# exoplanet-dev/celerite2

Measured on AMD Instinct MI355X. Metric: float64 GP log-lik+grad/sec at N=4096 J=8, batched, higher is better.
Workload: dtype f64; 1 GPU; configs[2]: batch of 65536 independent GPs (65536 per GPU), N=4096, J=8 (sum of 4 SHO terms), forward + reverse-mode grad, inputs resident in HBM; global_batch=65536, batch_per_gpu=65536, N=4096, J=8, parallelism=batch-sharded x1, all-gather of log-liks, failed_factorizations=0, clock_prewarm_steps=0

## Files before the change

### celerite2_amd/csrc/c2_loglik_t.hip

```cpp
#include <cstdint>
#include <cstdlib>
#include <type_traits>

#include "c2_loglik_helpers.hpp"
#include "../../include/celerite2_amd.h"

#ifndef C2T_J
#define C2T_J 8
#endif
#ifndef C2T_JS
#define C2T_JS C2T_J
#endif
#define C2T_CAT2(a, b) a##b
#define C2T_CAT(a, b) C2T_CAT2(a, b)
#define C2T_NAME(stem) C2T_CAT(stem, C2T_JS)
#define c2t C2T_CAT(c2t_j, C2T_JS)

namespace c2t {
using namespace c2;

constexpr int J = C2T_J;
static_assert(J == 8 || J == 4 || J == 2, "128-byte tiles of whole rows");
constexpr int NS = J * (J + 1) / 2;
constexpr int PPR = J / 2;
// ... 49 lines not shown
  __device__ __forceinline__ int rl(int i) const { const int s = (kWave / LPS) * i + lane / LPS; return (FULL || s < last) ? s : last; }
};
using RowIO = RowIOT<false>;

typedef double d2v __attribute__((ext_vector_type(2)));
__device__ __forceinline__ double2 ld2_in(const double2 *p) {
  const d2v v = __builtin_nontemporal_load(reinterpret_cast<const d2v *>(p));
  return make_double2(v.x, v.y);
}
__device__ __forceinline__ double ld1_in(const double *p) { return __builtin_nontemporal_load(p); }
template <class IO>
__device__ __forceinline__ void row_fetch(const double *__restrict__ base, int64_t N, int64_t n0, const IO &io,
                                          double (&st)[2 * NI]) {
  int64_t r = n0 + io.rpiece / PPR;
  r = r < 0 ? 0 : (r > N - 1 ? N - 1 : r);
  const int pc = piece_in(io.rpiece) ? io.rpiece % PPR : 0;
  const int64_t off = r * JS + 2 * pc;
#pragma unroll
  for (int i = 0; i < NI; ++i) {
    const double2 v = ld2_in(reinterpret_cast<const double2 *>(base + (int64_t)io.rl(i) * N * JS + off));
    st[2 * i] = piece_in(io.rpiece) ? v.x : 0.0; st[2 * i + 1] = piece_in(io.rpiece) ? v.y : 0.0;
  }
}
__device__ __forceinline__ void row_stage(double *tile, int lane, const double (&st)[2 * NI]) {
#pragma unroll
  for (int i = 0; i < NI; ++i)
    *reinterpret_cast<double2 *>(tile + ((kWave / LPS) * i + lane / LPS) * RSTR + 2 * (lane % LPS)) =
        make_double2(st[2 * i], st[2 * i + 1]);
}
__device__ __forceinline__ void row_read(const double *tile, int lane, int r, double (&x)[J]) {
#pragma unroll
  for (int q = 0; q < J / 2; ++q) {
    const double2 v = *reinterpret_cast<const double2 *>(tile + lane * RSTR + r * J + 2 * q);
    x[2 * q] = v.x; x[2 * q + 1] = v.y;
  }
}
__device__ __forceinline__ void row_write(double *tile, int lane, int r, const double (&x)[J]) {
#pragma unroll
  for (int q = 0; q < J / 2; ++q)
    *reinterpret_cast<double2 *>(tile + lane * RSTR + r * J + 2 * q) = make_double2(x[2 * q], x[2 * q + 1]);
}
__device__ __forceinline__ void row_flush(double *__restrict__ base, int64_t N, int64_t n0, int64_t lo, int64_t hi,
                                          const double *tile, int lane, int last) {
  const int piece = lane % LPS;
  const int64_t r = n0 + piece / PPR;
  if (last == kWave - 1 && n0 >= lo && n0 + RT - 1 <= hi) {
#pragma unroll
    for (int i = 0; i < NI; ++i) {
      const int s = (kWave / LPS) * i + lane / LPS;
      if (piece_in(piece))
        *reinterpret_cast<double2 *>(base + (int64_t)s * N * JS + r * JS + 2 * (piece % PPR)) =
            *reinterpret_cast<const double2 *>(tile + s * RSTR + 2 * piece);
    }
    return;
  }
#pragma unroll
  for (int i = 0; i < NI; ++i) {
    const int s = (kWave / LPS) * i + lane / LPS;
    const double2 v = *reinterpret_cast<const double2 *>(tile + s * RSTR + 2 * piece);
    if (s <= last && r >= lo && r <= hi && piece_in(piece))
      *reinterpret_cast<double2 *>(base + (int64_t)s * N * JS + r * JS + 2 * (piece % PPR)) = v;
  }
}

__device__ __forceinline__ void row_flush_full(double *__restrict__ base, int64_t N, int64_t n0, const double *tile,
                                               int lane) {
  const int piece = lane % LPS;
  const int64_t off = (n0 + piece / PPR) * JS + 2 * (piece % PPR);
#pragma unroll
  for (int i = 0; i < NI; ++i) {
    const int s = (kWave / LPS) * i + lane / LPS;
    if (piece_in(piece))
      *reinterpret_cast<double2 *>(base + (int64_t)s * N * JS + off) =
          *reinterpret_cast<const double2 *>(tile + s * RSTR + 2 * piece);
  }
}

__device__ __forceinline__ void sc_fetch(const double *__restrict__ base, int64_t N, int64_t n0, const RowIO &io,
                                         double (&st)[8]) {
  int64_t r = n0 + io.piece;
  r = r < 0 ? 0 : (r > N - 1 ? N - 1 : r);
#pragma unroll
  for (int i = 0; i < 8; ++i) st[i] = base[(int64_t)io.sl(i) * N + r];
}
__device__ __forceinline__ void sc_stage(double *tile, int lane, const double (&st)[8]) {
#pragma unroll
  for (int i = 0; i < 8; ++i) tile[(8 * i + lane / 8) * SSTR + (lane & 7)] = st[i];
}
__device__ __forceinline__ void sc_fetch16(const double *__restrict__ base, int64_t sN, int64_t N, int64_t n16, int lane,
                                           int last, double (&st)[16]) {
  int64_t r = n16 + (lane & 15);
  r = r < 0 ? 0 : (r > N - 1 ? N - 1 : r);
#pragma unroll
  for (int i = 0; i < 16; ++i) {
    const int s = 4 * i + lane / 16;
    st[i] = ld1_in(&base[(int64_t)(s < last ? s : last) * sN + r]);
  }
}
__device__ __forceinline__ void sc_stage16(double *tile, int lane, int half, const double (&st)[16]) {
  if (((lane & 15) >> 3) == half) {
#pragma unroll
    for (int i = 0; i < 16; ++i) tile[(4 * i + lane / 16) * SSTR + (lane & 7)] = st[i];
  }
}
__device__ __forceinline__ void sc_flush(double *__restrict__ base, int64_t N, int64_t n0, int64_t lo, int64_t hi,
                                         const double *tile, int lane, int last) {
  const int64_t r = n0 + (lane & 7);
  if (last == kWave - 1 && n0 >= lo && n0 + ST - 1 <= hi) {
    double v[8];
#pragma unroll
    for (int i = 0; i < 8; ++i) v[i] = tile[(8 * i + lane / 8) * SSTR + (lane & 7)];
    __builtin_amdgcn_sched_barrier(0);
#pragma unroll
    for (int i = 0; i < 8; ++i) base[(int64_t)(8 * i + lane / 8) * N + r] = v[i];
    return;
  }
#pragma unroll
  for (int i = 0; i < 8; ++i) {
    const int s = 8 * i + lane / 8;
    const double v = tile[s * SSTR + (lane & 7)];
    if (s <= last && r >= lo && r <= hi) base[(int64_t)s * N + r] = v;
  }
}

__device__ __forceinline__ void apark(double x, int &lo, int &hi) {
  asm volatile("v_accvgpr_write_b32 %0, %1" : "=a"(lo) : "v"(__double2loint(x)));
  asm volatile("v_accvgpr_write_b32 %0, %1" : "=a"(hi) : "v"(__double2hiint(x)));
}
template <int IMM>
__device__ __forceinline__ void aload(int &dst, const double *sbase, unsigned voff) {
  asm volatile("global_load_dword %0, %1, %2 offset:%3 nt" : "=a"(dst) : "v"(voff), "s"(sbase), "n"(IMM));
}
__device__ __forceinline__ void await_aloads() { asm volatile("s_waitcnt vmcnt(0)" ::: "memory"); }
__device__ __forceinline__ double afetch(int lo, int hi) {
  int l, h;
  asm volatile("v_accvgpr_read_b32 %0, %1" : "=v"(l) : "a"(lo));
  asm volatile("v_accvgpr_read_b32 %0, %1" : "=v"(h) : "a"(hi));
  return __hiloint2double(h, l);
}

#ifndef C2T_MLDS
#define C2T_MLDS 0
#endif
__device__ __forceinline__ double2 ld2_stream(const double2 *p) {
  const d2v v = __builtin_nontemporal_load(reinterpret_cast<const d2v *>(p));
  return make_double2(v.x, v.y);
}
__device__ __forceinline__ double ld1_stream(const double *p) { return __builtin_nontemporal_load(p); }
__device__ __forceinline__ void st2_stream(double2 *p, double2 v) {
  d2v w; w.x = v.x; w.y = v.y;
  __builtin_nontemporal_store(w, reinterpret_cast<d2v *>(p));
}
__device__ __forceinline__ void st1_stream(double *p, double v) { __builtin_nontemporal_store(v, p); }

template <bool PAIRED>
__device__ __forceinline__ void decay(const double (&c)[J], double dt, double (&p)[J]) {
  if constexpr (PAIRED) {
#pragma unroll
    for (int k = 0; k < J / 2; ++k) p[2 * k] = p[2 * k + 1] = exp_decay(c[2 * k] * dt);
  } else {
#pragma unroll
    for (int j = 0; j < J; ++j) p[j] = exp_decay(c[j] * dt);
  }
}

#ifdef C2T_PROF
__device__ unsigned long long c2t_prof[8];
#define C2T_TICK(k)                                                    \
  do {                                                                 \
    __builtin_amdgcn_sched_barrier(0);                                 \
    const unsigned long long now_ = __builtin_readcyclecounter();      \
    prof_[k] += now_ - tick_;                                          \
    tick_ = now_;                                                      \
    __builtin_amdgcn_sched_barrier(0);                                 \
  } while (0)
#else
#define C2T_TICK(k) do {} while (0)
#endif

struct TermsArgs {
  const double *ar, *cr, *ac, *bc, *cc, *dc;
  int batched;
};
template <int JC>
struct TermCoef {
  static constexpr int JR = J - 2 * (JC > 0 ? JC : 0);
  double ar[JR > 0 ? JR : 1], ac[JC > 0 ? JC : 1], bc[JC > 0 ? JC : 1], dc[JC > 0 ? JC : 1], A0;
  __device__ __forceinline__ void load(const TermsArgs &T, int64_t b, double (&cj)[J]) {
    const int64_t br = T.batched ? b * JR : 0, bk = T.batched ? b * JC : 0;
    double sum = 0.0;
#pragma unroll
    for (int r = 0; r < JR; ++r) { ar[r] = T.ar[br + r]; cj[r] = T.cr[br + r]; sum += ar[r]; }
#pragma unroll
    for (int k = 0; k < JC; ++k) {
      ac[k] = T.ac[bk + k]; bc[k] = T.bc[bk + k]; dc[k] = T.dc[bk + k];
      cj[JR + 2 * k] = cj[JR + 2 * k + 1] = T.cc[bk + k];
      sum += ac[k];
    }
    A0 = sum;
  }
  template <bool FAST>
  static __device__ __forceinline__ void sc(double ph, double &sn, double &cs) {
    if constexpr (FAST) sincos_cw_fast(ph, sn, cs);
    else sincos(ph, &sn, &cs);
  }
  __device__ __forceinline__ bool phases_fast(double x_first, double x_last) const {
    const double xm = fmax(fabs(x_first), fabs(x_last));
    bool ok = true;
#pragma unroll
    for (int k = 0; k < JC; ++k) ok = ok && (fabs(dc[k]) * xm < kSincosFastMax);
    return ok;
  }
  template <bool FAST>
  __device__ __forceinline__ void rows(double xn, double (&u)[J], double (&v)[J]) const {
#pragma unroll
    for (int r = 0; r < JR; ++r) { u[r] = ar[r]; v[r] = 1.0; }
#pragma unroll
    for (int k = 0; k < JC; ++k) {
      double sn, cs;
      sc<FAST>(dc[k] * xn, sn, cs);
      v[JR + 2 * k] = cs; v[JR + 2 * k + 1] = sn;
      u[JR + 2 * k] = fma(ac[k], cs, bc[k] * sn);
      u[JR + 2 * k + 1] = fma(ac[k], sn, -(bc[k] * cs));
    }
  }
  template <bool FAST>
  __device__ __forceinline__ void rows_sc(double xn, double (&u)[J], double (&sn)[JC > 0 ? JC : 1],
                                          double (&cs)[JC > 0 ? JC : 1]) const {
#pragma unroll
    for (int r = 0; r < JR; ++r) u[r] = ar[r];
#pragma unroll
    for (int k = 0; k < JC; ++k) {
      sc<FAST>(dc[k] * xn, sn[k], cs[k]);
      u[JR + 2 * k] = fma(ac[k], cs[k], bc[k] * sn[k]);
      u[JR + 2 * k + 1] = fma(ac[k], sn[k], -(bc[k] * cs[k]));
    }
  }
  __device__ __forceinline__ void decay(const double (&cj)[J], double dt, double (&p)[J]) const {
#pragma unroll
    for (int r = 0; r < JR; ++r) p[r] = exp_decay(cj[r] * dt);
#pragma unroll
    for (int k = 0; k < JC; ++k) p[JR + 2 * k] = p[JR + 2 * k + 1] = exp_decay(cj[JR + 2 * k] * dt);
  }
};

template <bool REC, bool PAIRED, int JC = -1, bool FAST = true>
__device__ __forceinline__ void fwd_body(int64_t B, int64_t N, const double *__restrict__ t, int64_t t_bs,
                                         const double *__restrict__ c, int64_t c_bs, const double *__restrict__ a,
                                         const double *__restrict__ U, const double *__restrict__ V,
                                         const double *__restrict__ y, double *__restrict__ ll,
                                         int32_t *__restrict__ flag, double *__restrict__ rec, Rec R,
                                         unsigned long long *__restrict__ guard, double *lds,
                                         const TermsArgs T = TermsArgs{}) {
  constexpr bool TERMS = JC >= 0;
  const int lane = threadIdx.x;
  const int64_t b0 = (int64_t)blockIdx.x * kWave;
  const int last = (int)((B - 1 - b0) < (kWave - 1) ? (B - 1 - b0) : (kWave - 1));
  const int sl = lane < last ? lane : last;
  const int64_t b = b0 + sl;
  const RowIO io(lane, last);
  double *tU = lds, *tV = tU + kWave * RSTR, *tT = tV + kWave * RSTR, *tA = tT + kWave * SSTR, *tY = tA + kWave * SSTR;
  const double *Ub = U + b0 * N * JS, *Vb = V + b0 * N * JS, *ab = a + b0 * N, *yb = y + b0 * N;
  const double *tb = t + (t_bs ? b0 * N : 0);
  const int64_t tN = t_bs ? N : 0;

  double cj[J];
  TermCoef<JC> tc;
  if constexpr (TERMS) tc.load(T, b, cj);
  else {
#pragma unroll
    for (int j = 0; j < J; ++j) cj[j] = j < JS ? c[b * c_bs + j] : 0.0;
  }
  double cmax = 0.0;
#pragma unroll
  for (int j = 0; j < J; ++j) cmax = fmax(cmax, cj[j]);

  constexpr size_t rsW = (size_t)(J / 2) * kWave, rs1 = kWave;
  double2 *recW = REC ? reinterpret_cast<double2 *>(rec + R.w + (size_t)blockIdx.x * N * J * kWave) : nullptr;
  double2 *recDZ = REC ? reinterpret_cast<double2 *>(rec + R.dz + (size_t)blockIdx.x * N * 2 * kWave) : nullptr;
  double *recCK = REC ? rec + R.ck + (size_t)blockIdx.x * R.nck * (NS + J) * kWave : nullptr;
  int32_t *recCKR = REC ? reinterpret_cast<int32_t *>(rec + R.ckr + (size_t)blockIdx.x * (((size_t)N + 1) / 2)) : nullptr;
  double *recT = REC ? rec + R.t + (size_t)blockIdx.x * N * kWave : nullptr;

  double S[NS];
#pragma unroll
  for (int k = 0; k < NS; ++k) S[k] = 0.0;
  double F[J], w[J];
  double tprev = t[b * t_bs];
  double d = a[b * N], z = y[b * N];
  if constexpr (TERMS) d += tc.A0;
  double rd = 1.0 / d;
  if constexpr (TERMS) {
    double u0[J], v0[J];
    tc.template rows<FAST>(tprev, u0, v0);
#pragma unroll
    for (int j = 0; j < J; ++j) { F[j] = 0.0; w[j] = v0[j] * rd; }
  } else {
#pragma unroll
    for (int j = 0; j < J; ++j) { F[j] = 0.0; w[j] = j < JS ? V[b * N * JS + j] * rd : 0.0; }
  }
  double prod = d, quad = z * z * rd;
  int eacc = 0;
  int32_t fl = 0;
  int slot = 0, nextra = 0;
  int64_t lastck = 0;
  auto write_ckpt = [&](int64_t row) __attribute__((always_inline)) {
// ... 92 lines not shown
            for (int j2 = 0; j2 < J; ++j2) w[j2] = (v[j2] - tau[j2]) * rd;
            fl = ((fl == 0) & (d <= 0.0)) ? (int32_t)n : fl;
            prod *= d;
            quad = fma(z * z, rd, quad);
            if (r & 1) { int e; prod = frexp(prod, &e); eacc += e; }
            if (REC) {
#pragma unroll
              for (int q = 0; q < J / 2; ++q) st2_stream(&recW[(size_t)n * rsW + q * kWave + lane], make_double2(w[2 * q], w[2 * q + 1]));
              const bool seg_end = (n % C == 0) || (n == N - 1);
              st2_stream(&recDZ[(size_t)n * rs1 + lane], make_double2(seg_end ? -fabs(d) : fabs(d), z));
              st1_stream(&recT[(size_t)n * rs1 + lane], tn);
              if (seg_end) write_ckpt(n);
            }
          }
        }
      }
    }
  }
  if (lane <= last) {
    int e;
    prod = frexp(prod, &e);
    const double logdet = log(prod) + (double)(eacc + e) * kLn2;
    flag[b] = fl;
    ll[b] = fl ? -INFINITY : -0.5 * (logdet + (double)N * kLog2Pi) - 0.5 * quad;
    if (REC && lane == 0) recCKR[0] = nextra;
  }
  if (REC) {
    double g = (gmax == gmax) ? gmax : INFINITY;
#pragma unroll
    for (int sft = 1; sft < kWave; sft <<= 1) g = fmax(g, __shfl_xor(g, sft, kWave));
    if (lane == 0) {
      const unsigned long long bits = (unsigned long long)__double_as_longlong(g);
      guard[kGateHeadWords + blockIdx.x] = bits;
      atomicMax(guard, bits);
      if (g > kGuard) atomicAdd(guard + 1, 1ull);
    }
  }
}

constexpr int kFwdLds = (2 * kWave * RSTR + 3 * kWave * SSTR) * 8;

template <bool REC>
__global__ __launch_bounds__(kWave, 1) void k_loglik_t_fwd(int64_t B, int64_t N, const double *__restrict__ t,
                                                           int64_t t_bs, const double *__restrict__ c, int64_t c_bs,
                                                           const double *__restrict__ a, const double *__restrict__ U,
                                                           const double *__restrict__ V, const double *__restrict__ y,
                                                           double *__restrict__ ll, int32_t *__restrict__ flag,
                                                           double *__restrict__ rec, Rec R,
                                                           unsigned long long *__restrict__ guard) {
  __shared__ __attribute__((aligned(16))) double lds[kFwdLds / 8];
  const int lane = threadIdx.x;
  const int64_t b0 = (int64_t)blockIdx.x * kWave;
  const int64_t bb = (b0 + lane) < B ? (b0 + lane) : (B - 1);
  bool paired = true;
#pragma unroll
  for (int k = 0; k < JS / 2; ++k) paired = paired && (c[bb * c_bs + 2 * k] == c[bb * c_bs + 2 * k + 1]);
  if (__all(paired))
    fwd_body<REC, true>(B, N, t, t_bs, c, c_bs, a, U, V, y, ll, flag, rec, R, guard, lds);
  else
    fwd_body<REC, false>(B, N, t, t_bs, c, c_bs, a, U, V, y, ll, flag, rec, R, guard, lds);
}

template <int JC>
__device__ __forceinline__ bool terms_phases_fast(int64_t B, int64_t N, const double *__restrict__ x, int64_t x_bs,
                                                  const TermsArgs &T) {
  const int64_t b0 = (int64_t)blockIdx.x * kWave;
  const int64_t b = (b0 + threadIdx.x) < B ? (b0 + threadIdx.x) : (B - 1);
  TermCoef<JC> tc;
  double cj[J];
  tc.load(T, b, cj);
  return __all(tc.phases_fast(x[b * x_bs], x[b * x_bs + N - 1]));
}

template <int JC, bool REC>
__global__ __launch_bounds__(kWave, 1) void k_loglik_tt_fwd(int64_t B, int64_t N, const double *__restrict__ t,
                                                            int64_t t_bs, TermsArgs T, const double *__restrict__ diag,
                                                            const double *__restrict__ y, double *__restrict__ ll,
                                                            int32_t *__restrict__ flag, double *__restrict__ rec, Rec R,
                                                            unsigned long long *__restrict__ guard) {
  __shared__ __attribute__((aligned(16))) double lds[kFwdLds / 8];
  if (terms_phases_fast<JC>(B, N, t, t_bs, T))
    fwd_body<REC, true, JC, true>(B, N, t, t_bs, nullptr, 0, diag, nullptr, nullptr, y, ll, flag, rec, R, guard, lds, T);
  else
    fwd_body<REC, true, JC, false>(B, N, t, t_bs, nullptr, 0, diag, nullptr, nullptr, y, ll, flag, rec, R, guard, lds, T);
}

constexpr int RS1 = J + 2;
constexpr int CS4 = 6;
constexpr int kRevLds = (2 * kWave * RSTR + 3 * kWave * SSTR + kWave * CS4 + kWave * RS1) * 8;
static_assert(kRevLds <= 40960 && (kWave * RSTR + kWave * RS1 + 3 * kWave * SSTR + 2 * kWave * RS1) * 8 <= kRevLds, "four wavefronts per CU");

__device__ __forceinline__ void row1_read(const double *tile, int lane, double (&x)[J]) {
#pragma unroll
  for (int q = 0; q < J / 2; ++q) {
    const double2 v = *reinterpret_cast<const double2 *>(tile + lane * RS1 + 2 * q);
    x[2 * q] = v.x; x[2 * q + 1] = v.y;
  }
}
__device__ __forceinline__ void row1_write(double *tile, int lane, const double (&x)[J]) {
#pragma unroll
  for (int q = 0; q < J / 2; ++q)
    *reinterpret_cast<double2 *>(tile + lane * RS1 + 2 * q) = make_double2(x[2 * q], x[2 * q + 1]);
}
__device__ __forceinline__ void row1_flush(double *__restrict__ base, int64_t N, int64_t n, const double *tile, int lane,
                                           int last) {
#pragma unroll
  for (int i = 0; i < PPR; ++i) {
    int sr = (kWave / PPR) * i + lane / PPR; sr = sr < last ? sr : last;
    if (piece_in(lane % PPR))
      *reinterpret_cast<double2 *>(base + ((int64_t)sr * N + n) * JS + 2 * (lane % PPR)) =
          *reinterpret_cast<const double2 *>(tile + sr * RS1 + 2 * (lane % PPR));
  }
}

struct TermsGrads {
  double *bar, *bcr, *bac, *bbc, *bcc, *bdc;
};
constexpr int AS1 = 14;

template <int K, class Step>
__device__ __forceinline__ void for_phases(Step &step, int64_t ntop, int64_t nf) {
  if constexpr (K >= 0) {
    const int64_t m = ntop - (RT - 1 - K);
    if (m <= nf && m >= 1) step(m, std::integral_constant<int, K>{});
    for_phases<K - 1>(step, ntop, nf);
  }
}

template <bool PAIRED, int JC = -1, bool FAST = true, bool FULL = false, bool XCK = false>
__device__ __forceinline__ void rev_body(int64_t B, int64_t N, const double *__restrict__ t, int64_t t_bs,
                                         const double *__restrict__ c, int64_t c_bs, const double *__restrict__ U,
                                         const int32_t *__restrict__ flag, const double *__restrict__ rec, Rec R,
                                         double *__restrict__ bt, double *__restrict__ bc, double *__restrict__ ba,
                                         double *__restrict__ bU, double *__restrict__ bV, double *__restrict__ by,
                                         double *lds, const TermsArgs T = TermsArgs{}, const TermsGrads G = TermsGrads{}) {
  constexpr bool TERMS = JC >= 0;
  constexpr int JR = TermCoef<JC>::JR, JCN = JC > 0 ? JC : 1;
  constexpr int NACC = TERMS ? JR + 3 * JC + 1 : 1;
  static_assert(NACC <= AS1, "accumulator tile");
  const int lane = threadIdx.x;
  const int64_t b0 = (int64_t)blockIdx.x * kWave;
  const int last = (int)((B - 1 - b0) < (kWave - 1) ? (B - 1 - b0) : (kWave - 1));
  const int sl = lane < last ? lane : last;
  const int64_t b = b0 + sl;
  const RowIOT<FULL> io(lane, last);
  constexpr bool BVPAIR = PAIRED && !TERMS;
  constexpr int CSTR = BVPAIR ? CS4 : RS1;
  double *tU = lds, *tBV = tU + kWave * RSTR, *tBA = tBV + kWave * (BVPAIR ? RSTR : RS1), *tBY = tBA + kWave * SSTR,
         *tBT = tBY + kWave * SSTR, *tC = tBT + kWave * SSTR, *tBC = tC + kWave * CSTR;
  static_assert((kWave * RSTR + kWave * (BVPAIR ? RSTR : RS1) + 3 * kWave * SSTR + kWave * CSTR + kWave * RS1) * 8 <= kRevLds, "LDS");
  double *tACC = lds;
  const double *Ub = U + b0 * N * JS;
  double *bUb = bU + b0 * N * JS, *bVb = bV + b0 * N * JS, *bab = ba + b0 * N, *byb = by + b0 * N, *btb = bt + b0 * N;
  constexpr size_t rsW = (size_t)(J / 2) * kWave, rs1 = kWave;
  const double2 *recW = reinterpret_cast<const double2 *>(rec + R.w + (size_t)blockIdx.x * N * J * kWave);
  const double2 *recDZ = reinterpret_cast<const double2 *>(rec + R.dz + (size_t)blockIdx.x * N * 2 * kWave);
  const double *recCK = rec + R.ck + (size_t)blockIdx.x * R.nck * (NS + J) * kWave;
  const int32_t *recCKR = reinterpret_cast<const int32_t *>(rec + R.ckr + (size_t)blockIdx.x * (((size_t)N + 1) / 2));
  const double *recT = rec + R.t + (size_t)blockIdx.x * N * kWave;
  const bool failed = flag[b] != 0;
  const double nan = __builtin_nan("");

  TermCoef<JC> tc;
  {
    double cj[J], zero[J];
    if constexpr (TERMS) tc.load(T, b, cj);
    else {
#pragma unroll
      for (int j = 0; j < J; ++j) cj[j] = j < JS ? c[b * c_bs + j] : 0.0;
    }
#pragma unroll
    for (int j = 0; j < J; ++j) zero[j] = 0.0;
    if constexpr (BVPAIR) {
#pragma unroll
      for (int k = 0; k < PPR; k += 2)
        *reinterpret_cast<double2 *>(tC + lane * CS4 + k) = make_double2(cj[2 * k], cj[2 * k + 2 < J ? 2 * k + 2 : 2 * k]);
    } else {
      row1_write(tC, lane, cj);
    }
    row1_write(tBC, lane, zero);
    if constexpr (TERMS) {
#pragma unroll
      for (int q = 0; q < AS1 / 2; ++q) *reinterpret_cast<double2 *>(tACC + lane * AS1 + 2 * q) = make_double2(0.0, 0.0);
    }
  }
  auto read_rates = [&](double (&cj)[J]) __attribute__((always_inline)) {
    if constexpr (BVPAIR) {
#pragma unroll
      for (int k = 0; k < PPR; k += 2) {
        const double2 c2k = *reinterpret_cast<const double2 *>(tC + lane * CS4 + k);
        cj[2 * k] = cj[2 * k + 1] = c2k.x;
        if (2 * k + 2 < J) cj[2 * k + 2] = cj[2 * k + 3] = c2k.y;
      }
    } else {
      row1_read(tC, lane, cj);
    }
  };
  auto accumulate = [&](const double (&u)[J], const double (&bu)[J], const double (&sn)[JCN], const double (&cs)[JCN],
                        const double (&gv)[JCN], double ba_n, double xn) -> double {
    double acc[AS1];
#pragma unroll
    for (int q = 0; q < AS1 / 2; ++q) {
      const double2 v = *reinterpret_cast<const double2 *>(tACC + lane * AS1 + 2 * q);
      acc[2 * q] = v.x; acc[2 * q + 1] = v.y;
    }
    double gsum = 0.0;
#pragma unroll
    for (int r = 0; r < JR; ++r) acc[r] += bu[r];
#pragma unroll
    for (int k = 0; k < JC; ++k) {
      const double b0_ = bu[JR + 2 * k], b1_ = bu[JR + 2 * k + 1];
      acc[JR + 3 * k] = fma(b0_, cs[k], fma(b1_, sn[k], acc[JR + 3 * k]));
      acc[JR + 3 * k + 1] = fma(b0_, sn[k], fma(-b1_, cs[k], acc[JR + 3 * k + 1]));
      const double g = fma(-b0_, u[JR + 2 * k + 1], fma(b1_, u[JR + 2 * k], gv[k]));
      acc[JR + 3 * k + 2] = fma(g, xn, acc[JR + 3 * k + 2]);
      gsum = fma(g, tc.dc[k], gsum);
    }
    acc[NACC - 1] += ba_n;
#pragma unroll
    for (int q = 0; q < AS1 / 2; ++q)
      *reinterpret_cast<double2 *>(tACC + lane * AS1 + 2 * q) = make_double2(acc[2 * q], acc[2 * q + 1]);
    return gsum;
  };

  double F[J], bF[J], bVn[J];
  int Slo[NS], Shi[NS], Mlo[NS], Mhi[NS];
#pragma unroll
  for (int k = 0; k < NS; ++k) { apark(0.0, Slo[k], Shi[k]); apark(0.0, Mlo[k], Mhi[k]); }
  constexpr int NML = (TERMS && C2T_MLDS && NS >= 18) ? 18 : 0;
  auto mslot = [&](int q) -> double2 * {
    return reinterpret_cast<double2 *>(lds + (q < 7 ? kWave * AS1 + q * 2 * kWave : kRevLds / 8 - (9 - q) * 2 * kWave)) + lane;
  };
  static_assert(NML == 0 || kWave * AS1 + 7 * 2 * kWave <= kWave * RSTR + kWave * RS1, "free LDS behind the accumulator tile");
  if constexpr (NML > 0) {
#pragma unroll
    for (int q = 0; q < NML / 2; ++q) *mslot(q) = make_double2(0.0, 0.0);
  }
  double2 mpair = make_double2(0.0, 0.0);
#pragma unroll
  for (int j = 0; j < J; ++j) { F[j] = 0.0; bF[j] = 0.0; bVn[j] = failed ? nan : 0.0; }
  double carry = 0.0;

  const double2 dzl = recDZ[(size_t)(N - 1) * rs1 + lane];
  const double rdl = 1.0 / fabs(dzl.x);
  double ban = 0.5 * rdl * (dzl.y * dzl.y * rdl - 1.0), bzn = -dzl.y * rdl;
  if (failed) { ban = nan; bzn = nan; }
  double tcur = recT[(size_t)(N - 1) * rs1 + lane];

  auto load_ckpt = [&](int64_t row) {
    const int64_t slot = XCK ? (int64_t)__builtin_amdgcn_readfirstlane(recCKR[row])
                             : ((row % C == 0) ? row / C - 1 : R.nreg - 1);
    const double *ck = recCK + (size_t)slot * (NS + J) * kWave;
    const unsigned voff = (unsigned)lane * 8u;
#pragma unroll
    for (int k = 0; k < NS; ++k) {
      const double *base = ck + (k / 8) * 8 * kWave;
      if ((k & 7) == 0) { aload<0>(Slo[k], base, voff); aload<4>(Shi[k], base, voff); }
      if ((k & 7) == 1) { aload<512>(Slo[k], base, voff); aload<516>(Shi[k], base, voff); }
      if ((k & 7) == 2) { aload<1024>(Slo[k], base, voff); aload<1028>(Shi[k], base, voff); }
      if ((k & 7) == 3) { aload<1536>(Slo[k], base, voff); aload<1540>(Shi[k], base, voff); }
      if ((k & 7) == 4) { aload<2048>(Slo[k], base, voff); aload<2052>(Shi[k], base, voff); }
      if ((k & 7) == 5) { aload<2560>(Slo[k], base, voff); aload<2564>(Shi[k], base, voff); }
      if ((k & 7) == 6) { aload<3072>(Slo[k], base, voff); aload<3076>(Shi[k], base, voff); }
      if ((k & 7) == 7) { aload<3584>(Slo[k], base, voff); aload<3588>(Shi[k], base, voff); }
    }
#pragma unroll
    for (int j = 0; j < J; ++j) F[j] = ld1_stream(&ck[(NS + j) * kWave + lane]);
    await_aloads();
  };
  auto t_fetch = [&](int64_t row) { return ld1_stream(&recT[(size_t)(row < 0 ? 0 : row) * rs1 + lane]); };
  auto w_fetch = [&](int64_t row, double (&wv)[J]) {
    row = row < 0 ? 0 : row;
#pragma unroll
    for (int q = 0; q < J / 2; ++q) {
      const double2 v = ld2_stream(&recW[(size_t)row * rsW + q * kWave + lane]);
      wv[2 * q] = v.x; wv[2 * q + 1] = v.y;
    }
  };
  auto dz_fetch = [&](int64_t row) { return ld2_stream(&recDZ[(size_t)(row < 0 ? 0 : row) * rs1 + lane]); };

  if (N >= 2) {
    const int64_t nf = N - 1;
    const int ph0 = (int)(nf % RT);
    const bool bv_seed_waits = BVPAIR && ph0 != 0;
    if constexpr (!TERMS) {
      if (bv_seed_waits) row_write(tBV, lane, ph0, bVn);
      else row1_write(tBV, lane, bVn);
    }
    tBA[lane * SSTR + (nf & (ST - 1))] = ban;
    tBY[lane * SSTR + (nf & (ST - 1))] = bzn;
    lds_order();
    if constexpr (!TERMS) {
      if (!bv_seed_waits) row1_flush(bVb, N, nf, tBV, lane, last);
    }
    if ((nf & (ST - 1)) == 0) {
      sc_flush(bab, N, nf, nf, nf, tBA, lane, last);
      sc_flush(byb, N, nf, nf, nf, tBY, lane, last);
    }
    double su[2 * NI];
    double wa[J];
    double2 dza;
    double ta;
    if constexpr (!TERMS) {
      row_fetch(Ub, N, nf - ph0, io, su);
      if (ph0 != RT - 1) {
        lds_order();
        row_stage(tU, lane, su);
        lds_order();
        row_fetch(Ub, N, nf - ph0 - RT, io, su);
      }
    }
    w_fetch(nf - 1, wa);
    dza = dz_fetch(nf - 1);
    ta = t_fetch(nf - 1);
    load_ckpt(nf);
    lds_order();

#ifdef C2T_PROF
    unsigned long long prof_[6] = {0, 0, 0, 0, 0, 0}, tick_ = __builtin_readcyclecounter();
#endif
    auto step = [&](const int64_t n, auto phase_tag) __attribute__((always_inline)) {
      constexpr int PH = decltype(phase_tag)::value;
      constexpr bool STAGE = PH == RT - 1;
      constexpr bool BUOUT = PH == 0;
      constexpr bool BVOUT = PH == (1 % RT);
      __builtin_amdgcn_sched_barrier(0);
      C2T_TICK(4);
      double wb[J];
      if constexpr (!TERMS && STAGE) {
        lds_order();
        row_stage(tU, lane, su);
        row_fetch(Ub, N, n - 2 * RT + 1, io, su);
      }
      w_fetch(n - 2, wb);
      const double2 dzb = dz_fetch(n - 2);
      const double tb2 = t_fetch(n - 2);
      if constexpr (!TERMS && STAGE) lds_order();

      const int rs = (int)((n - 1) & (ST - 1));
      double u[J], p[J], ip[J];
      double sn[JCN], cs[JCN], gv[JCN];
      const double xn = tcur;
      if constexpr (TERMS) {
        tc.template rows_sc<FAST>(xn, u, sn, cs);
#pragma unroll
        for (int k = 0; k < JC; ++k) gv[k] = fma(bVn[JR + 2 * k + 1], cs[k], -(bVn[JR + 2 * k] * sn[k]));
      } else {
        row_read(tU, lane, PH, u);
      }
      const double ba_in = ban;
      const double tm = ta;
      const double dt = tm - tcur;
      tcur = tm;
      {
        double cj[J];
        read_rates(cj);
        if constexpr (TERMS) tc.decay(cj, dt, p);
        else decay<PAIRED>(cj, dt, p);
      }
      C2T_TICK(0);
      double bp[J];
#pragma unroll
      for (int j = 0; j < J; ++j) {
        bF[j] = fma(-u[j], bzn, bF[j]);
        bp[j] = F[j] * bF[j];
        bF[j] *= p[j];
      }
      const double dm = fabs(dza.x), rdm = rcp_nr(dm), zm = dza.y;
      bool ckm = false;
      if constexpr (XCK) ckm = __builtin_amdgcn_readfirstlane(__double2hiint(dza.x)) < 0;
      double x[J];
      double xs[J], q[J];
      const double ba2 = 2.0 * ban;
#pragma unroll
      for (int j = 0; j < J; ++j) { x[j] = fma(ba2, u[j], bVn[j]); xs[j] = 0.0; q[j] = 0.0; ip[j] = rcp_nr(p[j]); }
#pragma unroll
      for (int i = 0; i < J; ++i) {
        const double dwi = dm * wa[i];
#pragma unroll
        for (int j2 = i; j2 < J; ++j2) {
          const int k = sidx(i, j2);
          const double sv = afetch(Slo[k], Shi[k]);
          double m;
          if (k < NML) {
            if ((k & 1) == 0) mpair = *mslot(k / 2);
            m = (k & 1) ? mpair.y : mpair.x;
          } else {
            m = afetch(Mlo[k], Mhi[k]);
          }
          xs[j2] = fma(x[i], sv, xs[j2]);
          if (j2 != i) xs[i] = fma(x[j2], sv, xs[i]);
          m = fma(-u[i], bVn[j2], m);
          m = fma(-x[i], u[j2], m);
          bp[j2] = fma(sv, m, bp[j2]);
          if (j2 != i) bp[i] = fma(sv, m, bp[i]);
          m *= p[i] * p[j2];
          if (k < NML) {
            if (k & 1) { mpair.y = m; *mslot(k / 2) = mpair; } else mpair.x = m;
          } else {
            apark(m, Mlo[k], Mhi[k]);
          }
          q[j2] = fma(wa[i], m, q[j2]);
          if (j2 != i) q[i] = fma(wa[j2], m, q[i]);
          apark(fma(-dwi, wa[j2], sv * (ip[i] * ip[j2])), Slo[k], Shi[k]);
        }
      }
      C2T_TICK(1);
      double gsum = 0.0;
      {
        double o[J];
#pragma unroll
        for (int j = 0; j < J; ++j) o[j] = fma(-bzn, F[j], -xs[j]);
        if constexpr (TERMS) gsum = accumulate(u, o, sn, cs, gv, ba_in, xn);
        else row_write(tU, lane, PH, o);
      }
      double f = 0.0;
      {
        double cj[J], bcj[J];
        read_rates(cj);
        row1_read(tBC, lane, bcj);
#pragma unroll
        for (int j = 0; j < J; ++j) { bcj[j] = fma(dt, bp[j], bcj[j]); f = fma(cj[j], bp[j], f); }
        row1_write(tBC, lane, bcj);
      }
      const double btn = carry - f + gsum;
      carry = f;
#pragma unroll
      for (int j = 0; j < J; ++j) F[j] = fma(-wa[j], zm, F[j] * ip[j]);
      double Gs = 0.0, Q = 0.0;
#pragma unroll
      for (int j = 0; j < J; ++j) { Gs = fma(wa[j], bF[j], Gs); Q = fma(q[j], wa[j], Q); }
      const double zr = zm * rdm;
      bzn = Gs - zr;
#pragma unroll
      for (int j = 0; j < J; ++j) bVn[j] = fma(zr, bF[j], q[j]);
      ban = 0.5 * rdm * (zm * zr - 1.0) - 0.5 * Q - zr * Gs;
      tBA[lane * SSTR + rs] = ban;
      tBY[lane * SSTR + rs] = bzn;
      tBT[lane * SSTR + (int)(n & (ST - 1))] = btn;
      if constexpr (BVPAIR) row_write(tBV, lane, (PH + RT - 1) % RT, bVn);
      else if constexpr (!TERMS) row1_write(tBV, lane, bVn);
      lds_order();
      if constexpr (!TERMS) {
        double fv[16], fu[16];
        if constexpr (!BVPAIR) {
#pragma unroll
          for (int i = 0; i < PPR; ++i) {
            int sr = (kWave / PPR) * i + lane / PPR; sr = (FULL || sr < last) ? sr : last;
            const double2 v1 = *reinterpret_cast<const double2 *>(tBV + sr * RS1 + 2 * (lane % PPR));
            fv[2 * i] = v1.x; fv[2 * i + 1] = v1.y;
          }
        } else if constexpr (BVOUT) {
#pragma unroll
          for (int i = 0; i < 8; ++i) {
            int sr = 8 * i + lane / 8; sr = (FULL || sr < last) ? sr : last;
            const double2 v1 = *reinterpret_cast<const double2 *>(tBV + sr * RSTR + 2 * (lane & 7));
            fv[2 * i] = v1.x; fv[2 * i + 1] = v1.y;
          }
        }
        if constexpr (BUOUT) {
#pragma unroll
          for (int i = 0; i < 8; ++i) {
            int sr = 8 * i + lane / 8; sr = (FULL || sr < last) ? sr : last;
            const double2 v0 = *reinterpret_cast<const double2 *>(tU + sr * RSTR + 2 * (lane & 7));
            fu[2 * i] = v0.x; fu[2 * i + 1] = v0.y;
          }
        }
        __builtin_amdgcn_sched_barrier(0);
        if constexpr (!BVPAIR) {
#pragma unroll
          for (int i = 0; i < PPR; ++i) {
            int sr = (kWave / PPR) * i + lane / PPR; sr = (FULL || sr < last) ? sr : last;
            if (piece_in(lane % PPR))
              st2_stream(reinterpret_cast<double2 *>(bVb + ((int64_t)sr * N + n - 1) * JS + 2 * (lane % PPR)), make_double2(fv[2 * i], fv[2 * i + 1]));
          }
        } else if constexpr (BVOUT) {
          if (RT == 2 || n - 1 + (lane & 7) / PPR <= nf) {
#pragma unroll
            for (int i = 0; i < 8; ++i) {
              int sr = 8 * i + lane / 8; sr = (FULL || sr < last) ? sr : last;
              if (piece_in(lane & 7))
                st2_stream(reinterpret_cast<double2 *>(bVb + ((int64_t)sr * N + n - 1) * JS + piece_off(lane & 7)), make_double2(fv[2 * i], fv[2 * i + 1]));
            }
          }
        }
        if constexpr (BUOUT) {
          if (n + (lane & 7) / PPR <= nf) {
#pragma unroll
            for (int i = 0; i < 8; ++i) {
              int sr = 8 * i + lane / 8; sr = (FULL || sr < last) ? sr : last;
              if (piece_in(lane & 7))
                st2_stream(reinterpret_cast<double2 *>(bUb + ((int64_t)sr * N + n) * JS + piece_off(lane & 7)), make_double2(fu[2 * i], fu[2 * i + 1]));
            }
          }
        }
      }

      C2T_TICK(2);
      if ((n & (ST - 1)) == 0) sc_flush(btb, N, n, 0, N - 1, tBT, lane, FULL ? kWave - 1 : last);
      if (rs == 0) {
        sc_flush(bab, N, n - 1, 0, N - 1, tBA, lane, FULL ? kWave - 1 : last);
        sc_flush(byb, N, n - 1, 0, N - 1, tBY, lane, FULL ? kWave - 1 : last);
        if constexpr (!XCK) { if (n >= 2 && (n - 1) % C == 0) load_ckpt(n - 1); }
      }
      if constexpr (XCK) { if (ckm && n >= 2) load_ckpt(n - 1); }
      C2T_TICK(5);
#pragma unroll
      for (int j = 0; j < J; ++j) wa[j] = wb[j];
      dza = dzb;
      ta = tb2;
      C2T_TICK(3);
    };
    if constexpr (TERMS) {
      for (int64_t n = nf; n >= 1; --n) step(n, std::integral_constant<int, 0>{});
    } else {
      if constexpr (RT == 2 && PAIRED) {
        for (int64_t n = nf | 1; n >= 1; n -= 2) {
          if (n <= nf) step(n, std::integral_constant<int, 1>{});
          if (n >= 2) step(n - 1, std::integral_constant<int, 0>{});
        }
      } else {
        for (int64_t ntop = nf | (RT - 1); ntop >= RT - 1; ntop -= RT) for_phases<RT - 1>(step, ntop, nf);
      }
    }
#ifdef C2T_PROF
    if (lane == 0 && blockIdx.x % 97 == 0)
      for (int k = 0; k < 6; ++k) atomicAdd(&c2t_prof[k], prof_[k]);
#endif
    {
      double zero[J];
#pragma unroll
      for (int j = 0; j < J; ++j) zero[j] = failed ? nan : 0.0;
      lds_order();
      if constexpr (TERMS) {
        double u0[J], sn[JCN], cs[JCN], gv[JCN], bu0[J];
        tc.template rows_sc<FAST>(tcur, u0, sn, cs);
#pragma unroll
        for (int j = 0; j < J; ++j) bu0[j] = 0.0;
#pragma unroll
        for (int k = 0; k < JC; ++k) gv[k] = fma(bVn[JR + 2 * k + 1], cs[k], -(bVn[JR + 2 * k] * sn[k]));
        carry += accumulate(u0, bu0, sn, cs, gv, ban, tcur);
      } else {
        row_write(tU, lane, 0, zero);
      }
      tBT[lane * SSTR] = carry;
      lds_order();
      if constexpr (!TERMS) {
        if ((lane & 7) / PPR <= nf) {
#pragma unroll
          for (int i = 0; i < 8; ++i) {
            int sr = 8 * i + lane / 8; sr = sr < last ? sr : last;
            if (piece_in(lane & 7))
              *reinterpret_cast<double2 *>(bUb + ((int64_t)sr * N) * JS + piece_off(lane & 7)) =
                  *reinterpret_cast<const double2 *>(tU + sr * RSTR + 2 * (lane & 7));
          }
        }
      }
      sc_flush(btb, N, 0, 0, (ST - 1) < (N - 1) ? (ST - 1) : (N - 1), tBT, lane, last);
    }
  } else {
    if (lane <= last) {
      bab[(int64_t)lane * N] = ban;
      byb[(int64_t)lane * N] = bzn;
      btb[(int64_t)lane * N] = failed ? nan : 0.0;
      if constexpr (TERMS) {
        tACC[lane * AS1 + NACC - 1] = ban;
        if (failed) {
          for (int q = 0; q < NACC; ++q) tACC[lane * AS1 + q] = nan;
          for (int j = 0; j < J; ++j) tBC[lane * RS1 + j] = nan;
        }
      } else {
#pragma unroll
        for (int j = 0; j < JS; ++j) { bUb[(int64_t)lane * N * JS + j] = failed ? nan : 0.0; bVb[(int64_t)lane * N * JS + j] = failed ? nan : 0.0; }
      }
    }
  }
  if (lane <= last) {
    double bcj[J];
    row1_read(tBC, lane, bcj);
    if constexpr (TERMS) {
      const double *acc = tACC + lane * AS1;
      const double sba = acc[NACC - 1];
#pragma unroll
      for (int r = 0; r < JR; ++r) { G.bar[b * JR + r] = sba + acc[r]; G.bcr[b * JR + r] = bcj[r]; }
#pragma unroll
      for (int k = 0; k < JC; ++k) {
        G.bac[b * JC + k] = sba + acc[JR + 3 * k];
        G.bbc[b * JC + k] = acc[JR + 3 * k + 1];
        G.bdc[b * JC + k] = acc[JR + 3 * k + 2];
        G.bcc[b * JC + k] = bcj[JR + 2 * k] + bcj[JR + 2 * k + 1];
      }
    } else {
#pragma unroll
      for (int j = 0; j < JS; ++j) bc[b * JS + j] = bcj[j];
    }
  }
}

__global__ __launch_bounds__(kWave, 1) void k_loglik_t_rev(int64_t B, int64_t N, const double *__restrict__ t,
                                                           int64_t t_bs, const double *__restrict__ c, int64_t c_bs,
                                                           const double *__restrict__ U,
                                                           const int32_t *__restrict__ flag,
                                                           const double *__restrict__ rec, Rec R,
                                                           const unsigned long long *__restrict__ guard,
                                                           double *__restrict__ bt, double *__restrict__ bc,
                                                           double *__restrict__ ba, double *__restrict__ bU,
                                                           double *__restrict__ bV, double *__restrict__ by) {
  __shared__ __attribute__((aligned(16))) double lds[kRevLds / 8];
  if (__longlong_as_double((long long)guard[kGateHeadWords + blockIdx.x]) > kGuard) return;
  const int lane = threadIdx.x;
  const int64_t b0 = (int64_t)blockIdx.x * kWave;
  const int64_t bb = (b0 + lane) < B ? (b0 + lane) : (B - 1);
  bool paired = true;
#pragma unroll
  for (int k = 0; k < JS / 2; ++k) paired = paired && (c[bb * c_bs + 2 * k] == c[bb * c_bs + 2 * k + 1]);
  const bool full = b0 + kWave <= B;
  const bool xck = __builtin_amdgcn_readfirstlane(
                       reinterpret_cast<const int32_t *>(rec + R.ckr + (size_t)blockIdx.x * (((size_t)N + 1) / 2))[0]) > 0;
#define C2T_REV(P_, F_, X_) rev_body<P_, -1, true, F_, X_>(B, N, t, t_bs, c, c_bs, U, flag, rec, R, bt, bc, ba, bU, bV, by, lds)
  if (__all(paired)) {
    if (full) { if (xck) C2T_REV(true, true, true); else C2T_REV(true, true, false); }
    else { if (xck) C2T_REV(true, false, true); else C2T_REV(true, false, false); }
  } else {
    if (full) { if (xck) C2T_REV(false, true, true); else C2T_REV(false, true, false); }
    else { if (xck) C2T_REV(false, false, true); else C2T_REV(false, false, false); }
  }
#undef C2T_REV
}

template <int JC>
__global__ __launch_bounds__(kWave, 1) void k_loglik_tt_rev(int64_t B, int64_t N, const double *__restrict__ x,
                                                            int64_t x_bs, TermsArgs T, const int32_t *__restrict__ flag,
                                                            const double *__restrict__ rec, Rec R,
                                                            const unsigned long long *__restrict__ guard, TermsGrads G,
                                                            double *__restrict__ bx, double *__restrict__ bdiag,
                                                            double *__restrict__ by) {
  __shared__ __attribute__((aligned(16))) double lds[kRevLds / 8];
  if (__longlong_as_double((long long)guard[kGateHeadWords + blockIdx.x]) > kGuard) return;
  const bool xck = __builtin_amdgcn_readfirstlane(
                       reinterpret_cast<const int32_t *>(rec + R.ckr + (size_t)blockIdx.x * (((size_t)N + 1) / 2))[0]) > 0;
#define C2T_TREV(FAST_, X_) rev_body<true, JC, FAST_, false, X_>(B, N, x, x_bs, nullptr, 0, nullptr, flag, rec, R, bx, nullptr, bdiag, nullptr, nullptr, by, lds, T, G)
  if (terms_phases_fast<JC>(B, N, x, x_bs, T)) { if (xck) C2T_TREV(true, true); else C2T_TREV(true, false); }
  else { if (xck) C2T_TREV(false, true); else C2T_TREV(false, false); }
#undef C2T_TREV
}

}

using namespace c2t;

extern "C" {

int C2T_NAME(c2_internal_loglik_t)(int64_t B, int64_t N, const double *t, int64_t t_bs, const double *c, int64_t c_bs,
                         const double *a, const double *U, const double *V, const double *y, double *ll,
                         int32_t *flag, c2_stream_t stream) {
  const dim3 grid((unsigned)((B + kWave - 1) / kWave));
  Rec R{};
  hipLaunchKernelGGL((k_loglik_t_fwd<false>), grid, dim3(kWave), 0, (hipStream_t)stream, B, N, t, t_bs, c, c_bs, a, U,
                     V, y, ll, flag, (double *)nullptr, R, (unsigned long long *)nullptr);
  return hipGetLastError() == hipSuccess ? C2_OK : C2_ERR_HIP;
}

size_t C2T_NAME(c2_internal_loglik_t_record_doubles)(int64_t B, int64_t N) { return rec_layout(B, N).total; }

int C2T_NAME(c2_internal_loglik_t_grad)(int64_t B, int64_t N, const double *t, int64_t t_bs, const double *c, int64_t c_bs,
                              const double *a, const double *U, const double *V, const double *y, double *ll,
                              double *bt, double *bc, double *ba, double *bU, double *bV, double *by, int32_t *flag,
                              double *rec, unsigned long long *guard, c2_stream_t stream) {
  const dim3 grid((unsigned)((B + kWave - 1) / kWave));
  const Rec R = rec_layout(B, N);
  hipStream_t s = (hipStream_t)stream;
  hipLaunchKernelGGL((k_loglik_t_fwd<true>), grid, dim3(kWave), 0, s, B, N, t, t_bs, c, c_bs, a, U, V, y, ll, flag, rec,
                     R, guard);
  if (hipGetLastError() != hipSuccess) return C2_ERR_HIP;
  hipLaunchKernelGGL(k_loglik_t_rev, grid, dim3(kWave), 0, s, B, N, t, t_bs, c, c_bs, U, (const int32_t *)flag,
                     (const double *)rec, R, (const unsigned long long *)guard, bt, bc, ba, bU, bV, by);
  return hipGetLastError() == hipSuccess ? C2_OK : C2_ERR_HIP;
}

int C2T_NAME(c2_internal_loglik_tt)(int64_t B, int64_t N, int64_t Jc, int coef_batched, const double *ar, const double *cr,
                          const double *ac, const double *bc, const double *cc, const double *dc, const double *x,
                          int64_t x_bs, const double *diag, const double *y, double *ll, int32_t *flag,
                          c2_stream_t stream) {
  const dim3 grid((unsigned)((B + kWave - 1) / kWave));
  const TermsArgs T{ar, cr, ac, bc, cc, dc, coef_batched};
  Rec R{};
#define C2_TT(JC_)                                                                                                       \
  hipLaunchKernelGGL((k_loglik_tt_fwd<JC_, false>), grid, dim3(kWave), 0, (hipStream_t)stream, B, N, x, x_bs, T, diag, y, \
                     ll, flag, (double *)nullptr, R, (unsigned long long *)nullptr)
  switch (Jc) {
#if C2T_JS == C2T_J
    case 0: C2_TT(0); break;
    case 1: C2_TT(1); break;
#endif
#if C2T_J >= 4 && C2T_JS == C2T_J
    case 2: C2_TT(2); break;
#endif
#if C2T_J >= 8 && C2T_JS == C2T_J
    case 3: C2_TT(3); break;
    case 4: C2_TT(4); break;
#endif
    default: return C2_ERR_UNSUPPORTED;
  }
#undef C2_TT
  return hipGetLastError() == hipSuccess ? C2_OK : C2_ERR_HIP;
}

int C2T_NAME(c2_internal_loglik_tt_grad)(int64_t B, int64_t N, int64_t Jc, int coef_batched, const double *ar, const double *cr,
                               const double *ac, const double *bc, const double *cc, const double *dc, const double *x,
                               int64_t x_bs, const double *diag, const double *y, double *ll, double *bar, double *bcr,
                               double *bac, double *bbc, double *bcc, double *bdc, double *bx, double *bdiag, double *by,
                               int32_t *flag, double *rec, unsigned long long *guard, c2_stream_t stream) {
  const dim3 grid((unsigned)((B + kWave - 1) / kWave));
  const TermsArgs T{ar, cr, ac, bc, cc, dc, coef_batched};
  const TermsGrads G{bar, bcr, bac, bbc, bcc, bdc};
  const Rec R = rec_layout(B, N);
  hipStream_t s = (hipStream_t)stream;
#define C2_TT(JC_)                                                                                                       \
  do {                                                                                                                   \
    hipLaunchKernelGGL((k_loglik_tt_fwd<JC_, true>), grid, dim3(kWave), 0, s, B, N, x, x_bs, T, diag, y, ll, flag, rec, R, \
                       guard);                                                                                           \
    if (hipGetLastError() != hipSuccess) return C2_ERR_HIP;                                                              \
    hipLaunchKernelGGL((k_loglik_tt_rev<JC_>), grid, dim3(kWave), 0, s, B, N, x, x_bs, T, (const int32_t *)flag,           \
                       (const double *)rec, R, (const unsigned long long *)guard, G, bx, bdiag, by);                     \
  } while (0)
  switch (Jc) {
#if C2T_JS == C2T_J
    case 0: C2_TT(0); break;
    case 1: C2_TT(1); break;
#endif
#if C2T_J >= 4 && C2T_JS == C2T_J
    case 2: C2_TT(2); break;
#endif
#if C2T_J >= 8 && C2T_JS == C2T_J
    case 3: C2_TT(3); break;
    case 4: C2_TT(4); break;
#endif
    default: return C2_ERR_UNSUPPORTED;
  }
#undef C2_TT
  return hipGetLastError() == hipSuccess ? C2_OK : C2_ERR_HIP;
}

#ifdef C2T_PROF
void c2_internal_prof_read(unsigned long long *out8) {
  hipDeviceSynchronize();
  hipMemcpyFromSymbol(out8, HIP_SYMBOL(c2t_prof), sizeof(unsigned long long) * 8);
  unsigned long long z[8] = {0, 0, 0, 0, 0, 0, 0, 0};
  hipMemcpyToSymbol(HIP_SYMBOL(c2t_prof), z, sizeof(z));
}
#endif

}
```

Before: 2.482 million GP/s.

## Use buffer-resource loads/stores with scalar offsets in reverse kernel for full wavefronts

Measured after the change: 2.505 million GP/s, median of 4. About the same (+0.9%).

```diff
diff --git a/celerite2_amd/csrc/c2_loglik_t.hip b/celerite2_amd/csrc/c2_loglik_t.hip
--- a/celerite2_amd/csrc/c2_loglik_t.hip
+++ b/celerite2_amd/csrc/c2_loglik_t.hip
@@ -225,6 +225,46 @@
   __builtin_nontemporal_store(w, reinterpret_cast<d2v *>(p));
 }
 __device__ __forceinline__ void st1_stream(double *p, double v) { __builtin_nontemporal_store(v, p); }
+
+typedef unsigned int u4v __attribute__((ext_vector_type(4)));
+typedef unsigned int u2v __attribute__((ext_vector_type(2)));
+using rsrc_t = __amdgpu_buffer_rsrc_t;
+constexpr int kAuxStream = 2;
+__host__ __device__ inline bool uniform_stretch(int64_t N) { return (uint64_t)N * J * kWave * 8 < (1ull << 31); }
+__device__ __forceinline__ rsrc_t stretch_of(const void *base, int64_t bytes) {
+  return __builtin_amdgcn_make_buffer_rsrc(const_cast<void *>(base), 0, (int)bytes, 0x00020000);
+}
+__device__ __forceinline__ double2 ld2_u(rsrc_t r, unsigned voff, int soff) {
+  const d2v v = __builtin_bit_cast(d2v, __builtin_amdgcn_raw_buffer_load_b128(r, (int)voff, soff, kAuxStream));
+  return make_double2(v.x, v.y);
+}
+__device__ __forceinline__ double ld1_u(rsrc_t r, unsigned voff, int soff) {
+  return __builtin_bit_cast(double, __builtin_amdgcn_raw_buffer_load_b64(r, (int)voff, soff, kAuxStream));
+}
+__device__ __forceinline__ void st2_u(rsrc_t r, unsigned voff, int soff, double2 v) {
+  d2v w; w.x = v.x; w.y = v.y;
+  __builtin_amdgcn_raw_buffer_store_b128(__builtin_bit_cast(u4v, w), r, (int)voff, soff, kAuxStream);
+}
+__device__ __forceinline__ void st1_u_cached(rsrc_t r, unsigned voff, int soff, double v) {
+  __builtin_amdgcn_raw_buffer_store_b64(__builtin_bit_cast(u2v, v), r, (int)voff, soff, 0);
+}
+__device__ __forceinline__ void row_fetch_u(rsrc_t r, unsigned voff, int soff, int tstride, int rpiece, double (&st)[2 * NI]) {
+#pragma unroll
+  for (int i = 0; i < NI; ++i) {
+    const double2 v = ld2_u(r, voff, soff + i * tstride);
+    st[2 * i] = piece_in(rpiece) ? v.x : 0.0; st[2 * i + 1] = piece_in(rpiece) ? v.y : 0.0;
+  }
+}
+__device__ __forceinline__ void sc_flush_u(rsrc_t r, unsigned voff, int soff, int tstride, bool rows_in, const double *tile, int lane) {
+  double v[8];
+#pragma unroll
+  for (int i = 0; i < 8; ++i) v[i] = tile[(8 * i + lane / 8) * SSTR + (lane & 7)];
+  __builtin_amdgcn_sched_barrier(0);
+  if (rows_in) {
+#pragma unroll
+    for (int i = 0; i < 8; ++i) st1_u_cached(r, voff, soff + i * tstride, v[i]);
+  }
+}
 
 template <bool PAIRED>
 __device__ __forceinline__ void decay(const double (&c)[J], double dt, double (&p)[J]) {
@@ -623,7 +663,7 @@
   double *tACC = lds;
   const double *Ub = U + b0 * N * JS;
   double *bUb = bU + b0 * N * JS, *bVb = bV + b0 * N * JS, *bab = ba + b0 * N, *byb = by + b0 * N, *btb = bt + b0 * N;
-  constexpr size_t rsW = (size_t)(J / 2) * kWave, rs1 = kWave;
+  constexpr size_t rowW = (size_t)(J / 2) * kWave, rs1 = kWave;
   const double2 *recW = reinterpret_cast<const double2 *>(rec + R.w + (size_t)blockIdx.x * N * J * kWave);
   const double2 *recDZ = reinterpret_cast<const double2 *>(rec + R.dz + (size_t)blockIdx.x * N * 2 * kWave);
   const double *recCK = rec + R.ck + (size_t)blockIdx.x * R.nck * (NS + J) * kWave;
@@ -631,6 +671,21 @@
   const double *recT = rec + R.t + (size_t)blockIdx.x * N * kWave;
   const bool failed = flag[b] != 0;
   const double nan = __builtin_nan("");
+  const int64_t NB = FULL ? N : 0;
+  const rsrc_t rsW = stretch_of(recW, NB * J * kWave * 8), rsDZ = stretch_of(recDZ, NB * 2 * kWave * 8), rsT = stretch_of(recT, NB * kWave * 8);
+  const rsrc_t rsU = stretch_of(Ub, NB * JS * kWave * 8), rsBU = stretch_of(bUb, NB * JS * kWave * 8), rsBV = stretch_of(bVb, NB * JS * kWave * 8);
+  const rsrc_t rsCK = stretch_of(recCK, FULL ? R.nck * (NS + J) * kWave * 8 : 0);
+  const rsrc_t rsBA = stretch_of(bab, NB * kWave * 8), rsBY = stretch_of(byb, NB * kWave * 8), rsBT = stretch_of(btb, NB * kWave * 8);
+  const int rstride = (int)(NB * JS * 8) * (kWave / LPS), sstride = (int)(NB * 8) * 8;
+  unsigned vo16 = (unsigned)lane * 16u, vo8 = (unsigned)lane * 8u;
+  unsigned voR = ((unsigned)(lane / LPS) * (unsigned)(NB * JS) + (unsigned)piece_off(piece_in(lane % LPS) ? lane % LPS : lane % LPS - lane % PPR)) * 8u;
+  unsigned voR1 = ((unsigned)(lane / PPR) * (unsigned)(NB * JS) + 2u * (unsigned)(lane % PPR)) * 8u;
+  unsigned voS = ((unsigned)(lane / 8) * (unsigned)NB + (unsigned)(lane & 7)) * 8u;
+  if constexpr (FULL) {
+    asm volatile("" : "+v"(vo16), "+v"(vo8), "+v"(voR), "+v"(voR1), "+v"(voS));
+  } else {
+    asm volatile("" : "+v"(vo16), "+v"(vo8));
+  }
 
   TermCoef<JC> tc;
   {
@@ -736,19 +791,30 @@
       if ((k & 7) == 7) { aload<3584>(Slo[k], base, voff); aload<3588>(Shi[k], base, voff); }
     }
 #pragma unroll
-    for (int j = 0; j < J; ++j) F[j] = ld1_stream(&ck[(NS + j) * kWave + lane]);
+    for (int j = 0; j < J; ++j) {
+      if constexpr (FULL) F[j] = ld1_u(rsCK, vo8, ((int)slot * (NS + J) + NS + j) * (kWave * 8));
+      else F[j] = ld1_u(stretch_of(ck + NS * kWave, J * kWave * 8), vo8, j * (kWave * 8));
+    }
     await_aloads();
   };
-  auto t_fetch = [&](int64_t row) { return ld1_stream(&recT[(size_t)(row < 0 ? 0 : row) * rs1 + lane]); };
+  auto t_fetch = [&](int64_t row) {
+    if constexpr (FULL) return ld1_u(rsT, vo8, (int)(row < 0 ? 0 : row) * (kWave * 8));
+    else return ld1_u(stretch_of(recT + (size_t)(row < 0 ? 0 : row) * rs1, kWave * 8), vo8, 0);
+  };
   auto w_fetch = [&](int64_t row, double (&wv)[J]) {
     row = row < 0 ? 0 : row;
 #pragma unroll
     for (int q = 0; q < J / 2; ++q) {
-      const double2 v = ld2_stream(&recW[(size_t)row * rsW + q * kWave + lane]);
+      double2 v;
+      if constexpr (FULL) v = ld2_u(rsW, vo16, (int)row * (int)(rowW * 16) + q * (kWave * 16));
+      else v = ld2_u(stretch_of(recW + (size_t)row * rowW, rowW * 16), vo16, q * (kWave * 16));
       wv[2 * q] = v.x; wv[2 * q + 1] = v.y;
     }
   };
-  auto dz_fetch = [&](int64_t row) { return ld2_stream(&recDZ[(size_t)(row < 0 ? 0 : row) * rs1 + lane]); };
+  auto dz_fetch = [&](int64_t row) {
+    if constexpr (FULL) return ld2_u(rsDZ, vo16, (int)(row < 0 ? 0 : row) * (kWave * 16));
+    else return ld2_u(stretch_of(recDZ + (size_t)(row < 0 ? 0 : row) * rs1, kWave * 16), vo16, 0);
+  };
 
   if (N >= 2) {
     const int64_t nf = N - 1;
@@ -801,7 +867,8 @@
       if constexpr (!TERMS && STAGE) {
         lds_order();
         row_stage(tU, lane, su);
-        row_fetch(Ub, N, n - 2 * RT + 1, io, su);
+        if constexpr (FULL) row_fetch_u(rsU, voR, (int)(n < 2 * RT - 1 ? 0 : n - 2 * RT + 1) * (JS * 8), rstride, io.rpiece, su);
+        else row_fetch(Ub, N, n - 2 * RT + 1, io, su);
       }
       w_fetch(n - 2, wb);
       const double2 dzb = dz_fetch(n - 2);
@@ -942,36 +1009,50 @@
 #pragma unroll
           for (int i = 0; i < PPR; ++i) {
             int sr = (kWave / PPR) * i + lane / PPR; sr = (FULL || sr < last) ? sr : last;
-            if (piece_in(lane % PPR))
-              st2_stream(reinterpret_cast<double2 *>(bVb + ((int64_t)sr * N + n - 1) * JS + 2 * (lane % PPR)), make_double2(fv[2 * i], fv[2 * i + 1]));
+            if (piece_in(lane % PPR)) {
+              if constexpr (FULL) st2_u(rsBV, voR1, (int)(n - 1) * (JS * 8) + i * ((int)(NB * JS * 8) * (kWave / PPR)), make_double2(fv[2 * i], fv[2 * i + 1]));
+              else st2_stream(reinterpret_cast<double2 *>(bVb + ((int64_t)sr * N + n - 1) * JS + 2 * (lane % PPR)), make_double2(fv[2 * i], fv[2 * i + 1]));
+            }
           }
         } else if constexpr (BVOUT) {
           if (RT == 2 || n - 1 + (lane & 7) / PPR <= nf) {
 #pragma unroll
             for (int i = 0; i < 8; ++i) {
               int sr = 8 * i + lane / 8; sr = (FULL || sr < last) ? sr : last;
-              if (piece_in(lane & 7))
-                st2_stream(reinterpret_cast<double2 *>(bVb + ((int64_t)sr * N + n - 1) * JS + piece_off(lane & 7)), make_double2(fv[2 * i], fv[2 * i + 1]));
+              if (piece_in(lane & 7)) {
+                if constexpr (FULL) st2_u(rsBV, voR, (int)(n - 1) * (JS * 8) + i * rstride, make_double2(fv[2 * i], fv[2 * i + 1]));
+                else st2_stream(reinterpret_cast<double2 *>(bVb + ((int64_t)sr * N + n - 1) * JS + piece_off(lane & 7)), make_double2(fv[2 * i], fv[2 * i + 1]));
+              }
             }
           }
         }
         if constexpr (BUOUT) {
-          if (n + (lane & 7) / PPR <= nf) {
+          if (FULL ? (lane & 7) / PPR <= (int)(nf - n) : n + (lane & 7) / PPR <= nf) {
 #pragma unroll
             for (int i = 0; i < 8; ++i) {
               int sr = 8 * i + lane / 8; sr = (FULL || sr < last) ? sr : last;
-              if (piece_in(lane & 7))
-                st2_stream(reinterpret_cast<double2 *>(bUb + ((int64_t)sr * N + n) * JS + piece_off(lane & 7)), make_double2(fu[2 * i], fu[2 * i + 1]));
+              if (piece_in(lane & 7)) {
+                if constexpr (FULL) st2_u(rsBU, voR, (int)n * (JS * 8) + i * rstride, make_double2(fu[2 * i], fu[2 * i + 1]));
+                else st2_stream(reinterpret_cast<double2 *>(bUb + ((int64_t)sr * N + n) * JS + piece_off(lane & 7)), make_double2(fu[2 * i], fu[2 * i + 1]));
+              }
             }
           }
         }
       }
 
       C2T_TICK(2);
-      if ((n & (ST - 1)) == 0) sc_flush(btb, N, n, 0, N - 1, tBT, lane, FULL ? kWave - 1 : last);
+      if ((n & (ST - 1)) == 0) {
+        if constexpr (FULL) sc_flush_u(rsBT, voS, (int)n * 8, sstride, (lane & 7) <= (int)(nf - n), tBT, lane);
+        else sc_flush(btb, N, n, 0, N - 1, tBT, lane, last);
+      }
       if (rs == 0) {
-        sc_flush(bab, N, n - 1, 0, N - 1, tBA, lane, FULL ? kWave - 1 : last);
-        sc_flush(byb, N, n - 1, 0, N - 1, tBY, lane, FULL ? kWave - 1 : last);
+        if constexpr (FULL) {
+          sc_flush_u(rsBA, voS, (int)(n - 1) * 8, sstride, (lane & 7) <= (int)(nf - n + 1), tBA, lane);
+          sc_flush_u(rsBY, voS, (int)(n - 1) * 8, sstride, (lane & 7) <= (int)(nf - n + 1), tBY, lane);
+        } else {
+          sc_flush(bab, N, n - 1, 0, N - 1, tBA, lane, last);
+          sc_flush(byb, N, n - 1, 0, N - 1, tBY, lane, last);
+        }
         if constexpr (!XCK) { if (n >= 2 && (n - 1) % C == 0) load_ckpt(n - 1); }
       }
       if constexpr (XCK) { if (ckm && n >= 2) load_ckpt(n - 1); }
@@ -1085,7 +1166,7 @@
   bool paired = true;
 #pragma unroll
   for (int k = 0; k < JS / 2; ++k) paired = paired && (c[bb * c_bs + 2 * k] == c[bb * c_bs + 2 * k + 1]);
-  const bool full = b0 + kWave <= B;
+  const bool full = b0 + kWave <= B && uniform_stretch(N);
   const bool xck = __builtin_amdgcn_readfirstlane(
                        reinterpret_cast<const int32_t *>(rec + R.ckr + (size_t)blockIdx.x * (((size_t)N + 1) / 2))[0]) > 0;
 #define C2T_REV(P_, F_, X_) rev_body<P_, -1, true, F_, X_>(B, N, t, t_bs, c, c_bs, U, flag, rec, R, bt, bc, ba, bU, bV, by, lds)
@@ -1133,6 +1214,8 @@
 }
 
 size_t C2T_NAME(c2_internal_loglik_t_record_doubles)(int64_t B, int64_t N) { return rec_layout(B, N).total; }
+
+int64_t C2T_NAME(c2_internal_loglik_t_rev_uniform_wavefronts)(int64_t B, int64_t N) { return uniform_stretch(N) ? B / kWave : 0; }
 
 int C2T_NAME(c2_internal_loglik_t_grad)(int64_t B, int64_t N, const double *t, int64_t t_bs, const double *c, int64_t c_bs,
                               const double *a, const double *U, const double *V, const double *y, double *ll,
```
